# elicassion/active-gym

Hardware: NVIDIA B200
Metric: foveal_obs_per_sec (higher is better)
Workload: dtype u8

## Files before the change

### active_gym_b200/csrc/agym_device.cuh

```cuda
#pragma once
#include "agym_kernels.cuh"
#ifndef AGYM_EXPERIMENT
#define AGYM_EXPERIMENT 0
#endif

#include <cuda.h>
#include <cuda_bf16.h>
#include <cuda_fp16.h>

#include <algorithm>
#include <utility>
#include <cstdlib>
#include <cstring>

#include "../../include/agym_b200.h"

namespace agym {

namespace {


constexpr int kThreads = 256;

__device__ __forceinline__ uint4 ld_stream128(const void *p) {
// ... 176 lines not shown
                "selp.u32 %0, 1, 0, p;\n\t}"
                : "=r"(done)
                : "r"(smem_u32(bar)), "r"(parity)
                : "memory");
        }
    }
}
__device__ __forceinline__ void bulk_g2s(void *smem_dst, const void *gmem_src, uint32_t bytes, uint64_t *bar) {
    asm volatile("cp.async.bulk.shared::cluster.global.mbarrier::complete_tx::bytes [%0], [%1], %2, [%3];" ::"r"(
                     smem_u32(smem_dst)),
                 "l"(gmem_src), "r"(bytes), "r"(smem_u32(bar))
                 : "memory");
}

__device__ __forceinline__ void tensor_g2s_4d(void *smem_dst, const CUtensorMap *map, uint64_t *bar, int c0, int c1, int c2, int c3) {
    asm volatile("cp.async.bulk.tensor.4d.shared::cluster.global.mbarrier::complete_tx::bytes [%0], [%1, {%3, %4, %5, %6}], [%2];" ::"r"(
                     smem_u32(smem_dst)),
                 "l"(reinterpret_cast<uint64_t>(map)), "r"(smem_u32(bar)), "r"(c0), "r"(c1), "r"(c2), "r"(c3)
                 : "memory");
}

__device__ __forceinline__ void bulk_s2g(void *gmem_dst, const void *smem_src, uint32_t bytes) {
    asm volatile("cp.async.bulk.global.shared::cta.bulk_group [%0], [%1], %2;" ::"l"(gmem_dst), "r"(smem_u32(smem_src)),
                 "r"(bytes)
                 : "memory");
}
__device__ __forceinline__ void bulk_commit() { asm volatile("cp.async.bulk.commit_group;" ::: "memory"); }
template <int N>
__device__ __forceinline__ void bulk_wait_read() { asm volatile("cp.async.bulk.wait_group.read %0;" ::"n"(N) : "memory"); }
__device__ __forceinline__ void fence_async_smem() { asm volatile("fence.proxy.async.shared::cta;" ::: "memory"); }

__device__ __forceinline__ void mbar_arrive(uint64_t *bar) {
    asm volatile("mbarrier.arrive.shared::cta.b64 _, [%0];" ::"r"(smem_u32(bar)) : "memory");
}
__device__ __forceinline__ void consumer_sync() { asm volatile("bar.sync 1, %0;" ::"n"(kThreads) : "memory"); }

__device__ __forceinline__ void pdl_launch_dependents() { asm volatile("griddepcontrol.launch_dependents;" ::: "memory"); }
__device__ __forceinline__ void pdl_wait() { asm volatile("griddepcontrol.wait;" ::: "memory"); }

__device__ __forceinline__ void cp_async16(void *smem_dst, const void *gmem_src) {
    asm volatile("cp.async.cg.shared.global [%0], [%1], 16;" ::"r"((uint32_t)__cvta_generic_to_shared(smem_dst)), "l"(gmem_src));
}
__device__ __forceinline__ void cp_async16_s(uint32_t smem_addr, const void *gmem_src) {
    asm volatile("cp.async.cg.shared.global [%0], [%1], 16;" ::"r"(smem_addr), "l"(gmem_src));
}
__device__ __forceinline__ void cp_async4(void *smem_dst, const void *gmem_src) {
    asm volatile("cp.async.ca.shared.global [%0], [%1], 4;" ::"r"((uint32_t)__cvta_generic_to_shared(smem_dst)), "l"(gmem_src));
}
__device__ __forceinline__ void cp_async4_s(uint32_t smem_addr, const void *gmem_src) {
    asm volatile("cp.async.ca.shared.global [%0], [%1], 4;" ::"r"(smem_addr), "l"(gmem_src));
}
template <int SOFF, int GOFF>
__device__ __forceinline__ void cp_async4_imm(uint32_t smem_addr, const void *gmem_src) {
    asm volatile("cp.async.ca.shared.global [%0 + %2], [%1 + %3], 4;" ::"r"(smem_addr), "l"(gmem_src), "n"(SOFF), "n"(GOFF));
}
__device__ __forceinline__ void cp_async_commit() { asm volatile("cp.async.commit_group;" ::: "memory"); }
template <int N>
__device__ __forceinline__ void cp_async_wait() { asm volatile("cp.async.wait_group %0;" ::"n"(N) : "memory"); }

__device__ __forceinline__ float norm_u8(uint32_t u) {
    const float x = (float)u, r = 1.0f / 255.0f;
    const float q0 = x * r;
    return fmaf(fmaf(-q0, 255.0f, x), r, q0);
}
__device__ __forceinline__ void norm_store4(int dt, uint32_t word, void *dst, size_t index) {
    const float f0 = norm_u8(word & 0xffu), f1 = norm_u8((word >> 8) & 0xffu), f2 = norm_u8((word >> 16) & 0xffu), f3 = norm_u8(word >> 24);
    if (dt == AGYM_DTYPE_F32) {
        reinterpret_cast<float4 *>(dst)[index] = make_float4(f0, f1, f2, f3);
    } else if (dt == AGYM_DTYPE_F16) {
        const __half2 a = __floats2half2_rn(f0, f1), b = __floats2half2_rn(f2, f3);
        reinterpret_cast<uint2 *>(dst)[index] = make_uint2(*reinterpret_cast<const uint32_t *>(&a), *reinterpret_cast<const uint32_t *>(&b));
    } else {
        const __nv_bfloat162 a = __floats2bfloat162_rn(f0, f1), b = __floats2bfloat162_rn(f2, f3);
        reinterpret_cast<uint2 *>(dst)[index] = make_uint2(*reinterpret_cast<const uint32_t *>(&a), *reinterpret_cast<const uint32_t *>(&b));
    }
}
__device__ __forceinline__ void norm_store16(int dt, const uint4 v, void *dst, size_t index) {
    const uint32_t w[4] = {v.x, v.y, v.z, v.w};
    if (dt == AGYM_DTYPE_F32) {
        float4 *o = reinterpret_cast<float4 *>(dst) + 4 * index;
#pragma unroll
        for (int j = 0; j < 4; ++j)
            o[j] = make_float4(norm_u8(w[j] & 0xffu), norm_u8((w[j] >> 8) & 0xffu), norm_u8((w[j] >> 16) & 0xffu), norm_u8(w[j] >> 24));
    } else {
        uint32_t h[8];
#pragma unroll
        for (int j = 0; j < 4; ++j) {
            const float f0 = norm_u8(w[j] & 0xffu), f1 = norm_u8((w[j] >> 8) & 0xffu), f2 = norm_u8((w[j] >> 16) & 0xffu), f3 = norm_u8(w[j] >> 24);
            if (dt == AGYM_DTYPE_F16) {
                const __half2 a = __floats2half2_rn(f0, f1), b = __floats2half2_rn(f2, f3);
                h[2 * j] = *reinterpret_cast<const uint32_t *>(&a); h[2 * j + 1] = *reinterpret_cast<const uint32_t *>(&b);
            } else {
                const __nv_bfloat162 a = __floats2bfloat162_rn(f0, f1), b = __floats2bfloat162_rn(f2, f3);
                h[2 * j] = *reinterpret_cast<const uint32_t *>(&a); h[2 * j + 1] = *reinterpret_cast<const uint32_t *>(&b);
            }
        }
        uint4 *o = reinterpret_cast<uint4 *>(dst) + 2 * index;
        o[0] = make_uint4(h[0], h[1], h[2], h[3]);
        o[1] = make_uint4(h[4], h[5], h[6], h[7]);
    }
}

__device__ __forceinline__ uint64_t pack2(float lo, float hi) {
    uint64_t r;
    asm("mov.b64 %0, {%1, %2};" : "=l"(r) : "f"(lo), "f"(hi));
    return r;
}
__device__ __forceinline__ void unpack2(uint64_t v, uint32_t &lo, uint32_t &hi) {
    asm("mov.b64 {%0, %1}, %2;" : "=r"(lo), "=r"(hi) : "l"(v));
}
__device__ __forceinline__ uint64_t ffma2(uint64_t a, uint64_t b, uint64_t c) {
    uint64_t d;
    asm("fma.rn.f32x2 %0, %1, %2, %3;" : "=l"(d) : "l"(a), "l"(b), "l"(c));
    return d;
}
__device__ __forceinline__ uint64_t fsub2(uint64_t a, uint64_t b) {
    uint64_t d;
    asm("sub.rn.f32x2 %0, %1, %2;" : "=l"(d) : "l"(a), "l"(b));
    return d;
}
__device__ __forceinline__ uint64_t fadd2(uint64_t a, uint64_t b) {
    uint64_t d;
    asm("add.rn.f32x2 %0, %1, %2;" : "=l"(d) : "l"(a), "l"(b));
    return d;
}

template <typename F>
cudaError_t set_smem(F func, size_t bytes) {
    if (bytes > 48 * 1024)
        return cudaFuncSetAttribute(func, cudaFuncAttributeMaxDynamicSharedMemorySize, (int)bytes);
    return cudaSuccess;
}

size_t a16(size_t v) { return (v + 15) & ~size_t(15); }

const bool g_no_pdl = getenv("AGYM_NO_PDL") != nullptr;

template <typename... KArgs, typename... Args>
cudaError_t launch_pdl(void (*kern)(KArgs...), dim3 grid, dim3 block, size_t smem, cudaStream_t st, Args &&...args) {
    cudaLaunchConfig_t cfg = {};
    cfg.gridDim = grid; cfg.blockDim = block; cfg.dynamicSmemBytes = smem; cfg.stream = st;
    cudaLaunchAttribute at[1];
    at[0].id = cudaLaunchAttributeProgrammaticStreamSerialization;
    at[0].val.programmaticStreamSerializationAllowed = g_no_pdl ? 0 : 1;
    cfg.attrs = at; cfg.numAttrs = 1;
    return cudaLaunchKernelEx(&cfg, kern, KArgs(std::forward<Args>(args))...);
}

const bool g_disable_std = getenv("AGYM_NO_STD") != nullptr;
const bool g_disable_tma = getenv("AGYM_NO_TMA") != nullptr;
const bool g_flex_old = getenv("AGYM_FLEX_OLD") != nullptr;
const bool g_crop_old = getenv("AGYM_CROP_OLD") != nullptr;
const bool g_crop_v2 = getenv("AGYM_CROP_V2") != nullptr;
const bool g_std_nofs = getenv("AGYM_STD_NOFS") != nullptr;
const int g_units = getenv("AGYM_INGEST_UNITS") ? atoi(getenv("AGYM_INGEST_UNITS")) : 0;


}

}
```

### active_gym_b200/csrc/agym_observe.cu

```cuda
#include "agym_device.cuh"

namespace agym {

namespace {

template <int VARIANT>
__global__ void __launch_bounds__(kThreads) k_observe_fixed(const __grid_constant__ DevPlan p,
                                                            const uint8_t *__restrict__ ring,
                                                            const int32_t *__restrict__ head,
                                                            const double *__restrict__ action,
                                                            const uint8_t *__restrict__ ctrl, int32_t *__restrict__ loc,
                                                            uint8_t *__restrict__ out) {
    extern __shared__ __align__(16) uint8_t smem[];
    __shared__ int s_loc[2];
    const int n = blockIdx.x, tid = threadIdx.x;
    if (tid == 0) {
        int r, c;
        update_loc_fixed(p, n, action, ctrl, loc, r, c);
        s_loc[0] = r; s_loc[1] = c;
    }
    __syncthreads();
    const int r0 = s_loc[0], c0 = s_loc[1];
    const int h = head[n];
    const uint8_t *env_ring = ring + (size_t)n * p.K * p.plane;
// ... 395 lines not shown
    const int nw_max = (p.f_w + 3) / 4 + 1;
    const int sq_words = (K * pp + 3) & ~3, buf_words = sq_words + ((K * f_h * nw_max + 3) & ~3);
    const int trows = K * p.p_h;
    float *bufs = reinterpret_cast<float *>(smem);
    float *s_T = bufs + 2 * buf_words;
    int2 *s_row = reinterpret_cast<int2 *>(s_T + trows * S_w);
    const uint32_t *ring_w = reinterpret_cast<const uint32_t *>(ring);
    uint32_t *out_w = reinterpret_cast<uint32_t *>(out);
    const int G = gridDim.x;

    const int npairs = S_w >> 1, parts = nt / npairs;
    const int a_part = tid / npairs, cp = tid - a_part * npairs;
    const bool a_active = a_part < parts;
    int a_i0 = 0, a_i1 = 0;
    uint64_t a_w0 = 0, a_w1 = 0;
    if (a_active) {
        a_i0 = __ldg(p.exw_i0 + 2 * cp);
        a_i1 = __ldg(p.exw_i0 + 2 * cp + 1);
        a_w0 = pack2(__ldg(p.exw_w0 + 2 * cp), __ldg(p.exw_w0 + 2 * cp + 1));
        a_w1 = pack2(__ldg(p.exw_w1 + 2 * cp), __ldg(p.exw_w1 + 2 * cp + 1));
    }
    const uint64_t bias2 = pack2(kBias, kBias);
    const int g = tid / quads, q = tid - g * quads;
    const bool active = g < ysegs;
    const int rows_per = (p.S_h + ysegs - 1) / ysegs;
    const int y_begin = g * rows_per, y_end = active ? min(p.S_h, y_begin + rows_per) : y_begin;
    const int pp4 = pp >> 2, frows = K * f_h;
    for (int i = tid; i < p.S_h; i += nt) s_row[i] = make_int2(__ldg(p.exh_i0 + i), __float_as_int(__ldg(p.exh_w0 + i)));
    if (tid == 0) s_row[p.S_h] = make_int2(-1, 0);

    auto issue = [&](int env, int lr, int lc, int hh, int b) {
        float *sq = bufs + b * buf_words;
        uint32_t *fv = reinterpret_cast<uint32_t *>(sq + sq_words);
        const size_t slot0 = (size_t)env * K;
        for (int k = 0; k < K; ++k) {
            int slot = hh + 1 + k;
            slot -= slot >= K ? K : 0;
            const float *src = pcache + (slot0 + slot) * pp;
            for (int c = tid; c < pp4; c += nt) cp_async16(sq + k * pp + 4 * c, src + 4 * c);
        }
        const int wq0 = lc >> 2, nw = ((lc + p.f_w - 1) >> 2) - wq0 + 1;
        for (int r = tid; r < frows; r += nt) {
            const int k = r / f_h, yy = r - k * f_h;
            int slot = hh + 1 + k;
            slot -= slot >= K ? K : 0;
            const uint32_t *src = ring_w + (slot0 + slot) * wpp + (uint32_t)(lr + yy) * quads + wq0;
            uint32_t *dst = fv + r * nw_max;
            for (int w = 0; w < nw; ++w) cp_async4(dst + w, src + w);
        }
    };
    auto next_loc = [&](int env, int slot) {
        int r = 0, c = 0;
        if (env < N) update_loc_fixed<true>(p, env, action, ctrl, loc, r, c);
        s_loc[slot][0] = r;
        s_loc[slot][1] = c;
    };

    int e = blockIdx.x;
    if (tid == 0) { next_loc(e, 0); next_loc(e + G, 1); }
    __syncthreads();
    int lr = s_loc[0][0], lc = s_loc[0][1], lr1 = s_loc[1][0], lc1 = s_loc[1][1];
    int hh = 0, hh1 = 0;
    if (e < N) { hh = head[e]; issue(e, lr, lc, hh, 0); }
    cp_async_commit();
    if (e + G < N) hh1 = head[e + G];
    __syncthreads();

    for (int it = 0; e < N; e += G, ++it) {
        const int en = e + G;
        if (en < N) issue(en, lr1, lc1, hh1, (it + 1) & 1);
        cp_async_commit();
        if (tid == 0) next_loc(en + G, it & 1);
        int hh2 = 0;
        if (en + G < N) hh2 = head[en + G];
        cp_async_wait<1>();
        __syncthreads();

        const float *sq = bufs + (it & 1) * buf_words;
        if (a_active) {
            const float *s = sq + a_part * p.p_w;
            float *t = s_T + a_part * S_w + 2 * cp;
            const int sstep = parts * p.p_w, tstep = parts * S_w;
#pragma unroll 4
            for (int r = a_part; r < trows; r += parts, s += sstep, t += tstep) {
                const uint64_t u = pack2(s[a_i0], s[a_i1]), v = pack2(s[a_i0 + 1], s[a_i1 + 1]);
                *reinterpret_cast<uint64_t *>(t) = ffma2(a_w0, u, ffma2(a_w1, v, bias2));
            }
        }
        __syncthreads();

        if (active) {
            const uint32_t *fvb = reinterpret_cast<const uint32_t *>(sq + sq_words);
            const uint32_t fov_mask = word_mask(4 * q, lc, lc + p.f_w);
            const int rf = fov_mask ? lr : (1 << 29);
            const int fstride = f_h * nw_max;
            for (int k0 = 0; k0 < K; k0 += KG) {
                uint32_t *orow = out_w + ((size_t)e * K + k0) * wpp + (uint32_t)y_begin * quads + q;
                const uint32_t *fv = fvb + (k0 * f_h - rf) * nw_max + (q - (lc >> 2));
                const float *tk = s_T + (size_t)k0 * p.p_h * S_w + 4 * q;
                const int kstride = p.p_h * S_w;
                int y = y_begin, j_have = -2;
                const int2 *rp = s_row + y_begin;
                int2 rw = *rp;
                uint64_t b0[KG], b1[KG], d0[KG], d1[KG];
                while (y < y_end) {
                    const int j0 = rw.x;
#pragma unroll
                    for (int kk = 0; kk < KG; ++kk) {
                        const float *tj = tk + kk * kstride + j0 * S_w;
                        uint64_t a0, a1;
                        if (j0 == j_have + 1) { a0 = b0[kk]; a1 = b1[kk]; }
                        else { const ulonglong2 a = *reinterpret_cast<const ulonglong2 *>(tj); a0 = a.x; a1 = a.y; }
                        const ulonglong2 b = *reinterpret_cast<const ulonglong2 *>(tj + S_w);
                        b0[kk] = b.x; b1[kk] = b.y;
                        d0[kk] = fsub2(a0, b.x); d1[kk] = fsub2(a1, b.y);
                    }
                    j_have = j0;
                    do {
                        const float w0 = __int_as_float(rw.y);
                        const uint64_t w2 = pack2(w0, w0);
                        rw = *++rp;
                        uint32_t word[KG];
#pragma unroll
                        for (int kk = 0; kk < KG; ++kk) {
                            uint32_t u0, u1, u2, u3;
                            unpack2(ffma2(w2, d0[kk], b0[kk]), u0, u1);
                            unpack2(ffma2(w2, d1[kk], b1[kk]), u2, u3);
                            word[kk] = __byte_perm(__byte_perm(u0, u1, 0x0051), __byte_perm(u2, u3, 0x0051), 0x5410);
                        }
                        if ((unsigned)(y - rf) < (unsigned)f_h) {
                            const uint32_t *sh = fv + y * nw_max;
#pragma unroll
                            for (int kk = 0; kk < KG; ++kk) word[kk] = (word[kk] & ~fov_mask) | (sh[kk * fstride] & fov_mask);
                        }
#pragma unroll
                        for (int kk = 0; kk < KG; ++kk) orow[kk * wpp] = word[kk];
                        orow += quads;
                        ++y;
                    } while (rw.x == j0 && y < y_end);
                }
            }
        }
        __syncthreads();
        lr = lr1; lc = lc1; hh = hh1; hh1 = hh2;
        lr1 = s_loc[it & 1][0]; lc1 = s_loc[it & 1][1];
    }
}

struct StdGeom {
    static constexpr int S = 84, P = 20, Q = 21, SEG = 4, R = 21, SPAN = 7;
    __host__ __device__ static constexpr int src(int i) { return (40 * i - 64 + 168 * 4) / 168 - 4; }
};

template <int NW, int R0>
__device__ __forceinline__ void prefetch_rows_imm(uint32_t rows, uint32_t dst, const uint32_t *src) {
    if constexpr (R0 < StdGeom::R) {
        if (rows & (1u << R0)) cp_async4_imm<R0 * (NW ? NW : 1) * 4, R0 * StdGeom::Q * 4>(dst, src);
        prefetch_rows_imm<NW, R0 + 1>(rows, dst, src);
    }
}

template <int K, int NW, bool FS>
__global__ void __launch_bounds__(((StdGeom::Q * StdGeom::SEG * K + 31) / 32) * 32, 2)
    k_observe_peripheral_std(const __grid_constant__ DevPlan p, const __grid_constant__ ExpandStd ew,
                             const uint8_t *__restrict__ ring, const int32_t *__restrict__ head,
                             const float *__restrict__ pcache, const double *__restrict__ action,
                             const uint8_t *__restrict__ ctrl, int32_t *__restrict__ loc, uint8_t *__restrict__ out) {
    using Gm = StdGeom;
    constexpr int S = Gm::S, P = Gm::P, Q = Gm::Q, R = Gm::R;
    constexpr int NB = Q * Gm::SEG * K;
    constexpr int PP = P * P, PLANE_W = S * S / 4;
    constexpr int NBUF = 3, DIST = 2, LOC_RING = 128;
    extern __shared__ __align__(16) uint8_t smem[];
    __shared__ int4 s_loc[LOC_RING];
    __shared__ __align__(8) uint64_t full[NBUF];
    const int tid = threadIdx.x;
    const int N = p.N, f_h = p.f_h, f_w = p.f_w, G = gridDim.x;
    const int nw_max = NW ? NW : (f_w + 3) / 4 + 1;
    const int rowbuf = (f_h * Q + 9) & ~3;
    const int buf_words = K * PP + (FS ? K * rowbuf : ((K * f_h * nw_max + 3) & ~3));
    float *bufs = reinterpret_cast<float *>(smem);
    uint32_t *tiles = reinterpret_cast<uint32_t *>(bufs + NBUF * buf_words);
    const uint32_t *ring_w = reinterpret_cast<const uint32_t *>(ring);

    auto loc_batch = [&](int it0) {
        const int j = it0 + (tid & 31);
        const int env = j <= N / G + 1 ? (int)blockIdx.x + j * G : N;
        int r = 0, c = 0, hh = 0;
        if (env < N) {
            update_loc_fixed<true>(p, env, action, ctrl, loc, r, c);
            hh = head[env];
        }
        s_loc[j & (LOC_RING - 1)] = make_int4(r, c, hh, 0);
    };
    pdl_launch_dependents();
    if (tid == 0) {
        for (int i = 0; i < NBUF; ++i) mbar_init(&full[i], 1);
        mbar_fence_init();
    }

    const bool active = tid < NB;
    const int q = tid % Q, t2 = tid / Q;
    constexpr int kOrd4[16] = {7, 4, 13, 3, 0, 1, 9, 6, 10, 14, 11, 12, 8, 5, 15, 2};
    constexpr int kOrd3[12] = {11, 8, 5, 2, 9, 6, 3, 0, 10, 4, 1, 7};
    const int grp = !active ? 0 : (K == 4 ? kOrd4[t2 & 15] : (K == 3 ? kOrd3[t2 % 12] : t2));
    const int g = grp % Gm::SEG, k = grp / Gm::SEG;
    int base;
    uint64_t wa01, wa23, wb01, wb23, wc01, wc23;
    {
        const int i00 = __ldg(p.exw_i0 + 4 * q);
        base = min(i00, P - 3);
        float wa[4], wb[4], wc[4];
#pragma unroll
        for (int c = 0; c < 4; ++c) {
            const int sel = __ldg(p.exw_i0 + 4 * q + c) - base;
            const float w0 = __ldg(p.exw_w0 + 4 * q + c), w1 = __ldg(p.exw_w1 + 4 * q + c);
            wa[c] = sel == 0 ? w0 : 0.f;
            wb[c] = sel == 0 ? w1 : w0;
            wc[c] = sel == 0 ? 0.f : w1;
        }
        wa01 = pack2(wa[0], wa[1]); wa23 = pack2(wa[2], wa[3]);
        wb01 = pack2(wb[0], wb[1]); wb23 = pack2(wb[2], wb[3]);
        wc01 = pack2(wc[0], wc[1]); wc23 = pack2(wc[2], wc[3]);
    }
    const uint64_t bias2 = pack2(kBias, kBias);
    const int row_first = 5 * g - 1;
    const int so_t0 = (row_first < 0 ? 0 : row_first) * P + base;
    const int so_mid = row_first * P + base;
    const int so_t6 = (row_first + 6 > P - 1 ? P - 1 : row_first + 6) * P + base;
    const uint32_t bufs_s = smem_u32(bufs);
    const uint32_t word0 = (uint32_t)(g * R) * Q + q;
    constexpr int NJ = 2;
    int ck_row[NJ], ck_k[NJ], ck_c4[NJ];
    if constexpr (FS) {
        const int cpr = (f_w + 14) / 16 + 1, total = K * f_h * cpr;
#pragma unroll
        for (int a = 0; a < NJ; ++a) {
            const int i = tid + a * (int)blockDim.x;
            const int row = i / cpr, kk = row / f_h;
            ck_k[a] = i < total ? kk : -1;
            ck_row[a] = (row - kk * f_h) * Q;
            ck_c4[a] = (i - row * cpr) * 4;
        }
    }

    auto fovea_rows = [&](int lr, int lc, uint32_t &mask) {
        mask = word_mask(4 * q, lc, lc + f_w);
        const int r_lo = lr - g * R;
        const int m_lo = max(r_lo, 0), m_hi = min(r_lo + f_h, R);
        return (mask && m_hi > m_lo) ? (((1u << m_hi) - 1u) & ~((1u << m_lo) - 1u)) : 0u;
    };
    auto fovea_pos = [&](int lr, int lc) { return (k * f_h + g * R - lr) * nw_max + (q - (lc >> 2)); };
    auto prefetch = [&](int env, int j) {
        const int b = j % NBUF;
        if (tid == 0) {
            mbar_expect_tx(&full[b], K * PP * 4);
            bulk_g2s(bufs + b * buf_words, pcache + (size_t)env * (K * PP), K * PP * 4, &full[b]);
        }
        if constexpr (FS) {
            const int4 lh = s_loc[j & (LOC_RING - 1)];
            const int top = lh.x * Q, wb = top & ~3;
            const int lw = lh.y >> 2, lastw = (lh.y + f_w - 1) >> 2;
#pragma unroll
            for (int a = 0; a < NJ; ++a) {
                if (ck_k[a] < 0) continue;
                const int rowbase = top + ck_row[a];
                const int cw = ((rowbase + lw) & ~3) + ck_c4[a];
                if (cw > rowbase + lastw) continue;
                int slot = lh.z + 1 + ck_k[a];
                slot -= slot >= K ? K : 0;
                cp_async16_s(bufs_s + (uint32_t)(b * buf_words + K * PP + ck_k[a] * rowbuf + (cw - wb)) * 4u,
                             ring_w + ((size_t)env * K + slot) * PLANE_W + cw);
            }
        } else if (active) {
            const int4 lh = s_loc[j & (LOC_RING - 1)];
            uint32_t mask;
            const uint32_t rows = fovea_rows(lh.x, lh.y, mask);
            if (rows) {
                int slot = lh.z + 1 + k;
                slot -= slot >= K ? K : 0;
                const uint32_t *src = ring_w + ((size_t)env * K + slot) * PLANE_W + word0;
                const uint32_t dst = bufs_s + (uint32_t)(b * buf_words + K * PP + fovea_pos(lh.x, lh.y)) * 4u;
                if (NW) {
                    prefetch_rows_imm<NW, 0>(rows, dst, src);
                } else {
#pragma unroll
                    for (int r = 0; r < R; ++r)
                        if (rows & (1u << r)) cp_async4_s(dst + (uint32_t)(r * nw_max) * 4u, src + r * Q);
                }
            }
        }
    };
    auto t_row = [&](const float *sq, int so, uint64_t &t01, uint64_t &t23) {
        const float s0 = sq[so], s1 = sq[so + 1], s2 = sq[so + 2];
        const uint64_t p0 = pack2(s0, s0), p1 = pack2(s1, s1), p2 = pack2(s2, s2);
        t01 = ffma2(p2, wc01, ffma2(p1, wb01, ffma2(p0, wa01, bias2)));
        t23 = ffma2(p2, wc23, ffma2(p1, wb23, ffma2(p0, wa23, bias2)));
    };

    pdl_wait();
    if (tid < 32) loc_batch(0);
    __syncthreads();
    {
        const int e0 = blockIdx.x;
#pragma unroll
        for (int j = 0; j < DIST; ++j) {
            if (e0 + j * G < N) prefetch(e0 + j * G, j);
            cp_async_commit();
        }
        if constexpr (FS) {
            cp_async_wait<DIST - 1>();
            __syncthreads();
        }
    }
    int it = 0;
    for (int e = blockIdx.x; e < N; e += G, ++it) {
        if (e + DIST * G < N) prefetch(e + DIST * G, it + DIST);
        cp_async_commit();
        if ((it & 31) == 0 && tid < 32) loc_batch(it + 32);
        const int b = it % NBUF;
        if constexpr (!FS) cp_async_wait<DIST>();
        mbar_wait(&full[b], (it / NBUF) & 1);
        uint32_t *tile = tiles + (it & 1) * (K * PLANE_W);
        if (active) {
            const int4 lh = s_loc[it & (LOC_RING - 1)];
            uint32_t fov_mask;
            const uint32_t rows = fovea_rows(lh.x, lh.y, fov_mask);
            int slot = lh.z + 1 + k;
            slot -= slot >= K ? K : 0;
            const float *sq = bufs + b * buf_words + slot * PP;
            const uint32_t *sh = reinterpret_cast<const uint32_t *>(bufs + b * buf_words + K * PP) +
                                 (FS ? k * rowbuf + (int)word0 - ((lh.x * Q) & ~3) : fovea_pos(lh.x, lh.y));
            constexpr int SHP = FS ? Q : 0;
            uint32_t *o = tile + k * PLANE_W + word0;
            uint64_t a0, a1, b0, b1, d0 = 0, d1 = 0;
            t_row(sq, so_t0, a0, a1);
            t_row(sq, so_mid + P, b0, b1);
            int t_have = 0;
#pragma unroll
            for (int r = 0; r < R; ++r) {
                const int t = Gm::src(r) + 1;
                if (t != t_have) {
                    a0 = b0; a1 = b1;
                    t_row(sq, t + 1 == Gm::SPAN - 1 ? so_t6 : so_mid + (t + 1) * P, b0, b1);
                    t_have = t;
                }
                if (r == 0 || Gm::src(r) != Gm::src(r - 1)) { d0 = fsub2(a0, b0); d1 = fsub2(a1, b1); }
                const uint64_t w2 = pack2(ew.hw[r], ew.hw[r]);
                uint32_t u0, u1, u2, u3;
                unpack2(ffma2(w2, d0, b0), u0, u1);
                unpack2(ffma2(w2, d1, b1), u2, u3);
                uint32_t word = __byte_perm(__byte_perm(u0, u1, 0x0051), __byte_perm(u2, u3, 0x0051), 0x5410);
                if (rows & (1u << r))
                    word = (word & ~fov_mask) | (sh[FS ? r * SHP : r * nw_max] & fov_mask);
                o[r * Q] = word;
            }
        }
        fence_async_smem();
        if (tid == 0) bulk_wait_read<0>();
        if constexpr (FS) cp_async_wait<DIST - 1>();
        __syncthreads();
        if (tid == 0) {
            bulk_s2g(out + (size_t)e * (K * PLANE_W * 4), tile, K * PLANE_W * 4);
            bulk_commit();
        }
        if (p.norm_out) {
            const uint4 *t4 = reinterpret_cast<const uint4 *>(tile);
            for (int i = tid; i < K * PLANE_W / 4; i += (int)blockDim.x)
                norm_store16(p.norm_dt, t4[i], p.norm_out, (size_t)e * (K * PLANE_W / 4) + i);
        }
    }
    if (tid == 0) bulk_wait_read<0>();
}


}

namespace {
cudaError_t normalize_after(cudaError_t e, const uint8_t *out, size_t bytes, void *norm_out, int norm_dt, cudaStream_t st) {
    if (e != cudaSuccess || !norm_out) return e;
    if (bytes % 16 != 0) return cudaErrorInvalidValue;
    return launch_normalize(out, bytes, norm_dt, norm_out, st);
}
}

cudaError_t launch_observe_fixed(const DevPlan &p0, const uint8_t *ring, const int32_t *head, const double *action,
                                 const uint8_t *ctrl, int32_t *loc, int variant, uint8_t *out, void *norm_out, int norm_dt,
                                 cudaStream_t st) {
    DevPlan p = p0;
    p.norm_out = norm_out; p.norm_dt = norm_dt;
    const size_t out_bytes = (size_t)p.N * p.K * (variant == AGYM_OUT_CROP ? p.f_h * p.f_w : p.plane);
    cudaError_t e;
    const int crop_nwx = (p.f_w + 2) / 4 + 1;
    const size_t crop_smem = a16((size_t)(p.K * p.f_h * p.f_w / 4) * 8) + (size_t)kCropWarps * p.K * p.f_h * crop_nwx * 4;
    CropV3Args c3;
    c3.nch = (p.f_w + 30) / 16;
    c3.g = p.f_w % 4 == 0 ? 1 : p.f_w % 2 == 0 ? 2 : 4;
    c3.gw = c3.g * p.f_w / 4;
    c3.ngroups = p.K * p.f_h / c3.g;
    c3.m_fh = 0xFFFFFFFFu / (uint32_t)p.f_h + 1u;
    c3.slice = (int)(16 + (size_t)p.K * p.f_h * c3.nch * 16);
    const int c3_warps = (p.C == 3 && (size_t)kCrop3Warps * (c3.slice + (size_t)p.K * p.f_h * p.f_w) > 100 * 1024) ? 4 : kCrop3Warps;
    const size_t crop3_smem = (size_t)c3_warps * (c3.slice + (size_t)p.K * p.f_h * p.f_w);
    if (variant == AGYM_OUT_CROP && (p.K * p.f_h * p.f_w) % 4 == 0 && (p.K * p.f_h) % c3.g == 0 && p.plane % 16 == 0 &&
        (reinterpret_cast<uintptr_t>(ring) & 15) == 0 && (reinterpret_cast<uintptr_t>(out) & 3) == 0 &&
        !g_disable_std && !g_crop_old && !g_crop_v2 && crop3_smem <= 100 * 1024) {
        const int grid = (p.N + c3_warps - 1) / c3_warps;
#define AGYM_LAUNCH_CROP3(FW, W)                                                                                  \
    {                                                                                                             \
        if ((e = set_smem(k_observe_fixed_crop_v3<FW, W>, crop3_smem)) != cudaSuccess) return e;                   \
        k_observe_fixed_crop_v3<FW, W><<<grid, W * 32, crop3_smem, st>>>(p, ring, head, action, ctrl, loc, out, c3); \
    }
        if (c3_warps == 4) {
            if (p.f_w == 30) AGYM_LAUNCH_CROP3(30, 4)
            else AGYM_LAUNCH_CROP3(0, 4)
        } else if (p.f_w == 30) AGYM_LAUNCH_CROP3(30, kCrop3Warps)
        else AGYM_LAUNCH_CROP3(0, kCrop3Warps)
#undef AGYM_LAUNCH_CROP3
        return cudaGetLastError();
    }
    if (variant == AGYM_OUT_CROP && (p.K * p.f_h * p.f_w) % 4 == 0 && !g_disable_std && !g_crop_old &&
        crop_smem <= 64 * 1024 && p.K * p.f_h * crop_nwx * 4 + 4 < 65536) {
        if ((e = set_smem(k_observe_fixed_crop_v2, crop_smem)) != cudaSuccess) return e;
        k_observe_fixed_crop_v2<<<(p.N + kCropWarps - 1) / kCropWarps, kCropWarps * 32, crop_smem, st>>>(p, ring, head, action, ctrl, loc, out, crop_nwx);
        return cudaGetLastError();
    } else if (variant == AGYM_OUT_CROP && (p.K * p.f_h * p.f_w) % 4 == 0 && !g_disable_std) {
        k_observe_fixed_crop_warp<<<(p.N + kThreads / 32 - 1) / (kThreads / 32), kThreads, 0, st>>>(p, ring, head, action, ctrl, loc, out);
    } else if (variant == AGYM_OUT_CROP) {
        k_observe_fixed<AGYM_OUT_CROP><<<p.N, kThreads, 0, st>>>(p, ring, head, action, ctrl, loc, out);
    } else if (variant == AGYM_OUT_MASK) {
        k_observe_fixed<AGYM_OUT_MASK><<<p.N, kThreads, 0, st>>>(p, ring, head, action, ctrl, loc, out);
    } else {
        const size_t smem = sizeof(float) * ((size_t)p.f_h * p.f_w + (size_t)p.f_h * p.S_w);
        if ((e = set_smem(k_observe_fixed<AGYM_OUT_RESIZE_FULL>, smem)) != cudaSuccess) return e;
        k_observe_fixed<AGYM_OUT_RESIZE_FULL><<<p.N, kThreads, smem, st>>>(p, ring, head, action, ctrl, loc, out);
    }
    return normalize_after(cudaGetLastError(), out, out_bytes, norm_out, norm_dt, st);
}

cudaError_t launch_observe_peripheral(const DevPlan &p0, const ExpandStd *ew, const uint8_t *ring, const int32_t *head,
                                      const float *pcache, const double *action, const uint8_t *ctrl, int32_t *loc,
                                      uint8_t *out, void *norm_out, int norm_dt, cudaStream_t st) {
    DevPlan p = p0;
    p.norm_out = norm_out; p.norm_dt = norm_dt;
    const size_t out_bytes = (size_t)p.N * p.K * p.plane;
    const size_t smem = a16(p.plane) + sizeof(float) * ((size_t)p.S_h * p.p_w + (size_t)p.p_h * p.p_w + (size_t)p.p_h * p.S_w);
    cudaError_t e;
    const int quads = p.S_w / 4;
    if (pcache && ew && ew->ok && (p.K == 4 || p.K == 3) && !g_disable_std && p.N < (1 << 30) &&
        (reinterpret_cast<uintptr_t>(out) & 15) == 0 && (reinterpret_cast<uintptr_t>(pcache) & 15) == 0) {
        const int nw_max = (p.f_w + 3) / 4 + 1;
        const size_t fov_words = ((size_t)p.K * p.f_h * nw_max + 3) & ~size_t(3);
        size_t fs = 4 * (3 * ((size_t)p.K * 400 + fov_words) + 2 * (size_t)p.K * 1764);
        const size_t fs_rows = 4 * (3 * ((size_t)p.K * 400 + (size_t)p.K * ((p.f_h * 21 + 9) & ~3)) + 2 * (size_t)p.K * 1764);
        const int std_threads = ((21 * 4 * p.K + 31) / 32) * 32;
        const bool full_rows = !g_std_nofs && fs_rows <= 112 * 1024 && p.K * p.f_h * ((p.f_w + 14) / 16 + 1) <= 2 * std_threads;
        int dev = 0, sms = 148, occ = 0;
        cudaGetDevice(&dev);
        cudaDeviceGetAttribute(&sms, cudaDevAttrMultiProcessorCount, dev);
#define AGYM_LAUNCH_STD(KK, NW, FSV)                                                                               \
    {                                                                                                              \
    if (fs <= 220 * 1024) {                                                                                        \
        const int threads = ((21 * 4 * KK + 31) / 32) * 32;                                                        \
        if ((e = set_smem(k_observe_peripheral_std<KK, NW, FSV>, fs)) != cudaSuccess) return e;                    \
        cudaOccupancyMaxActiveBlocksPerMultiprocessor(&occ, k_observe_peripheral_std<KK, NW, FSV>, threads, fs);   \
        if (occ >= 1) {                                                                                            \
            return launch_pdl(k_observe_peripheral_std<KK, NW, FSV>, dim3(std::min(p.N, sms * occ)), dim3(threads), fs, st, \
                              p, *ew, ring, head, pcache, action, ctrl, loc, out);                                 \
        }                                                                                                          \
    }                                                                                                              \
    }
        if (full_rows) {
            fs = fs_rows;
            if (p.K == 4) AGYM_LAUNCH_STD(4, 0, true)
            else AGYM_LAUNCH_STD(3, 0, true)
        }
        else if (p.K == 4 && nw_max == 9) AGYM_LAUNCH_STD(4, 9, false)
        else if (p.K == 4) AGYM_LAUNCH_STD(4, 0, false)
        else if (nw_max == 9) AGYM_LAUNCH_STD(3, 9, false)
        else AGYM_LAUNCH_STD(3, 0, false)
#undef AGYM_LAUNCH_STD
    }
    if (pcache && p.fast_expand && quads <= 64 && (p.p_h * p.p_w) % 4 == 0) {
        int ysegs = std::max(1, 128 / quads);
        {
            int g = p.S_h, b2 = p.p_h;
            while (b2) { const int t = g % b2; g = b2; b2 = t; }
            const int period = p.S_h / g;
            while (ysegs > 1 && (p.S_h % ysegs != 0 || (p.S_h / ysegs) % period != 0)) --ysegs;
        }
        const int threads = ((std::max(quads * ysegs, 2 * quads) + 31) / 32) * 32;
        const int nw_max = (p.f_w + 3) / 4 + 1;
        const size_t buf_words = (((size_t)p.K * p.p_h * p.p_w + 3) & ~size_t(3)) + (((size_t)p.K * p.f_h * nw_max + 3) & ~size_t(3));
        const size_t fs = 4 * (2 * buf_words + (size_t)p.K * p.p_h * p.S_w) + 8 * ((size_t)p.S_h + 1);
        int dev = 0, sms = 148, occ = 1;
        cudaGetDevice(&dev);
        cudaDeviceGetAttribute(&sms, cudaDevAttrMultiProcessorCount, dev);
#define AGYM_LAUNCH_PF(KG, PW)                                                                                     \
    {                                                                                                              \
        if ((e = set_smem(k_observe_peripheral_v2<KG, PW>, fs)) != cudaSuccess) return e;                          \
        cudaOccupancyMaxActiveBlocksPerMultiprocessor(&occ, k_observe_peripheral_v2<KG, PW>, threads, fs);         \
        if (occ < 1) return cudaErrorInvalidConfiguration;                                                         \
        k_observe_peripheral_v2<KG, PW><<<std::min(p.N, sms * occ), threads, fs, st>>>(p, ring, head, pcache, action, \
                                                                                      ctrl, loc, out, ysegs);     \
    }
        if (p.K == 4 && p.plane == 7056) AGYM_LAUNCH_PF(4, 1764)
        else if (p.K == 3 && p.plane == 7056) AGYM_LAUNCH_PF(3, 1764)
        else if (p.C == 3 && p.K % 3 == 0 && p.plane == 7056) AGYM_LAUNCH_PF(3, 1764)
        else if (p.K % 4 == 0) AGYM_LAUNCH_PF(4, 0)
        else if (p.K % 3 == 0) AGYM_LAUNCH_PF(3, 0)
        else if (p.K % 2 == 0) AGYM_LAUNCH_PF(2, 0)
        else AGYM_LAUNCH_PF(1, 0)
#undef AGYM_LAUNCH_PF
        return normalize_after(cudaGetLastError(), out, out_bytes, norm_out, norm_dt, st);
    }
    if (pcache) {
        if ((e = set_smem(k_observe_peripheral<true>, smem)) != cudaSuccess) return e;
        k_observe_peripheral<true><<<p.N, kThreads, smem, st>>>(p, ring, head, pcache, action, ctrl, loc, out);
    } else {
        if ((e = set_smem(k_observe_peripheral<false>, smem)) != cudaSuccess) return e;
        k_observe_peripheral<false><<<p.N, kThreads, smem, st>>>(p, ring, head, pcache, action, ctrl, loc, out);
    }
    return normalize_after(cudaGetLastError(), out, out_bytes, norm_out, norm_dt, st);
}


}
```

Before: 51.58 million.

## Replace per-env peripheral std kernel with per-plane 96-thread pipelined kernel

The templated per-environment kernel, which processed all K frame planes in one block of 21*4*K threads, is replaced by a single non-templated kernel. Each 96-thread block handles one plane at a time and runs a TMA and cp.async prefetch pipeline over (env, plane) pairs. This shrinks shared memory per block and allows up to 8 blocks per SM, and it extends the fast path to K=9 with C=3. Lanes are assigned to output words so that a warp's stores fall on distinct banks. The trade-offs are more pipeline stages and barriers per env, one bulk store per plane, and the PDL launch-dependents trigger moving to the end of the kernel, which may reduce overlap with the next kernel.

```diff
diff --git a/active_gym_b200/csrc/agym_device.cuh b/active_gym_b200/csrc/agym_device.cuh
--- a/active_gym_b200/csrc/agym_device.cuh
+++ b/active_gym_b200/csrc/agym_device.cuh
@@ -352,7 +352,6 @@
 const bool g_flex_old = getenv("AGYM_FLEX_OLD") != nullptr;
 const bool g_crop_old = getenv("AGYM_CROP_OLD") != nullptr;
 const bool g_crop_v2 = getenv("AGYM_CROP_V2") != nullptr;
-const bool g_std_nofs = getenv("AGYM_STD_NOFS") != nullptr;
 const int g_units = getenv("AGYM_INGEST_UNITS") ? atoi(getenv("AGYM_INGEST_UNITS")) : 0;
 
 
diff --git a/active_gym_b200/csrc/agym_observe.cu b/active_gym_b200/csrc/agym_observe.cu
--- a/active_gym_b200/csrc/agym_observe.cu
+++ b/active_gym_b200/csrc/agym_observe.cu
@@ -571,33 +571,23 @@
     __host__ __device__ static constexpr int src(int i) { return (40 * i - 64 + 168 * 4) / 168 - 4; }
 };
 
-template <int NW, int R0>
-__device__ __forceinline__ void prefetch_rows_imm(uint32_t rows, uint32_t dst, const uint32_t *src) {
-    if constexpr (R0 < StdGeom::R) {
-        if (rows & (1u << R0)) cp_async4_imm<R0 * (NW ? NW : 1) * 4, R0 * StdGeom::Q * 4>(dst, src);
-        prefetch_rows_imm<NW, R0 + 1>(rows, dst, src);
-    }
-}
-
-template <int K, int NW, bool FS>
-__global__ void __launch_bounds__(((StdGeom::Q * StdGeom::SEG * K + 31) / 32) * 32, 2)
-    k_observe_peripheral_std(const __grid_constant__ DevPlan p, const __grid_constant__ ExpandStd ew,
-                             const uint8_t *__restrict__ ring, const int32_t *__restrict__ head,
-                             const float *__restrict__ pcache, const double *__restrict__ action,
-                             const uint8_t *__restrict__ ctrl, int32_t *__restrict__ loc, uint8_t *__restrict__ out) {
+constexpr int kPlaneThreads = 96;
+__global__ void __launch_bounds__(kPlaneThreads, 8)
+    k_observe_peripheral_planes(const __grid_constant__ DevPlan p, const __grid_constant__ ExpandStd ew,
+                                const uint8_t *__restrict__ ring, const int32_t *__restrict__ head,
+                                const float *__restrict__ pcache, const double *__restrict__ action,
+                                const uint8_t *__restrict__ ctrl, int32_t *__restrict__ loc, uint8_t *__restrict__ out) {
     using Gm = StdGeom;
     constexpr int S = Gm::S, P = Gm::P, Q = Gm::Q, R = Gm::R;
-    constexpr int NB = Q * Gm::SEG * K;
     constexpr int PP = P * P, PLANE_W = S * S / 4;
-    constexpr int NBUF = 3, DIST = 2, LOC_RING = 128;
+    constexpr int NBUF = 3, DIST = 2, LOC_RING = 64;
     extern __shared__ __align__(16) uint8_t smem[];
     __shared__ int4 s_loc[LOC_RING];
     __shared__ __align__(8) uint64_t full[NBUF];
     const int tid = threadIdx.x;
-    const int N = p.N, f_h = p.f_h, f_w = p.f_w, G = gridDim.x;
-    const int nw_max = NW ? NW : (f_w + 3) / 4 + 1;
+    const int N = p.N, K = p.K, f_h = p.f_h, f_w = p.f_w, G = gridDim.x;
     const int rowbuf = (f_h * Q + 9) & ~3;
-    const int buf_words = K * PP + (FS ? K * rowbuf : ((K * f_h * nw_max + 3) & ~3));
+    const int buf_words = PP + rowbuf;
     float *bufs = reinterpret_cast<float *>(smem);
     uint32_t *tiles = reinterpret_cast<uint32_t *>(bufs + NBUF * buf_words);
     const uint32_t *ring_w = reinterpret_cast<const uint32_t *>(ring);
@@ -612,18 +602,21 @@
         }
         s_loc[j & (LOC_RING - 1)] = make_int4(r, c, hh, 0);
     };
-    pdl_launch_dependents();
     if (tid == 0) {
         for (int i = 0; i < NBUF; ++i) mbar_init(&full[i], 1);
         mbar_fence_init();
     }
 
-    const bool active = tid < NB;
-    const int q = tid % Q, t2 = tid / Q;
-    constexpr int kOrd4[16] = {7, 4, 13, 3, 0, 1, 9, 6, 10, 14, 11, 12, 8, 5, 15, 2};
-    constexpr int kOrd3[12] = {11, 8, 5, 2, 9, 6, 3, 0, 10, 4, 1, 7};
-    const int grp = !active ? 0 : (K == 4 ? kOrd4[t2 & 15] : (K == 3 ? kOrd3[t2 % 12] : t2));
-    const int g = grp % Gm::SEG, k = grp / Gm::SEG;
+    const int warp = tid >> 5, lane = tid & 31;
+    int item = -1;
+    {
+        int seen = 0;
+#pragma unroll
+        for (int i = 0; i < Q * Gm::SEG; ++i)
+            if ((i / Q * R * Q + i % Q) % 32 == lane && seen++ == warp) item = i;
+    }
+    const bool active = item >= 0;
+    const int q = active ? item % Q : 0, g = active ? item / Q : 0;
     int base;
     uint64_t wa01, wa23, wb01, wb23, wc01, wc23;
     {
@@ -649,19 +642,8 @@
     const int so_t6 = (row_first + 6 > P - 1 ? P - 1 : row_first + 6) * P + base;
     const uint32_t bufs_s = smem_u32(bufs);
     const uint32_t word0 = (uint32_t)(g * R) * Q + q;
-    constexpr int NJ = 2;
-    int ck_row[NJ], ck_k[NJ], ck_c4[NJ];
-    if constexpr (FS) {
-        const int cpr = (f_w + 14) / 16 + 1, total = K * f_h * cpr;
-#pragma unroll
-        for (int a = 0; a < NJ; ++a) {
-            const int i = tid + a * (int)blockDim.x;
-            const int row = i / cpr, kk = row / f_h;
-            ck_k[a] = i < total ? kk : -1;
-            ck_row[a] = (row - kk * f_h) * Q;
-            ck_c4[a] = (i - row * cpr) * 4;
-        }
-    }
+    const int cpr = (f_w + 14) / 16 + 1, chunks = f_h * cpr;
+    const FastDiv fd_cpr(cpr);
 
     auto fovea_rows = [&](int lr, int lc, uint32_t &mask) {
         mask = word_mask(4 * q, lc, lc + f_w);
@@ -669,45 +651,24 @@
         const int m_lo = max(r_lo, 0), m_hi = min(r_lo + f_h, R);
         return (mask && m_hi > m_lo) ? (((1u << m_hi) - 1u) & ~((1u << m_lo) - 1u)) : 0u;
     };
-    auto fovea_pos = [&](int lr, int lc) { return (k * f_h + g * R - lr) * nw_max + (q - (lc >> 2)); };
-    auto prefetch = [&](int env, int j) {
-        const int b = j % NBUF;
+    auto prefetch = [&](int ie, int k, int jb) {
+        const int b = jb % NBUF;
+        const int4 lh = s_loc[ie & (LOC_RING - 1)];
+        int slot = lh.z + 1 + k;
+        slot -= slot >= K ? K : 0;
+        const size_t plane = (size_t)((int)blockIdx.x + ie * G) * K + slot;
         if (tid == 0) {
-            mbar_expect_tx(&full[b], K * PP * 4);
-            bulk_g2s(bufs + b * buf_words, pcache + (size_t)env * (K * PP), K * PP * 4, &full[b]);
-        }
-        if constexpr (FS) {
-            const int4 lh = s_loc[j & (LOC_RING - 1)];
-            const int top = lh.x * Q, wb = top & ~3;
-            const int lw = lh.y >> 2, lastw = (lh.y + f_w - 1) >> 2;
-#pragma unroll
-            for (int a = 0; a < NJ; ++a) {
-                if (ck_k[a] < 0) continue;
-                const int rowbase = top + ck_row[a];
-                const int cw = ((rowbase + lw) & ~3) + ck_c4[a];
-                if (cw > rowbase + lastw) continue;
-                int slot = lh.z + 1 + ck_k[a];
-                slot -= slot >= K ? K : 0;
-                cp_async16_s(bufs_s + (uint32_t)(b * buf_words + K * PP + ck_k[a] * rowbuf + (cw - wb)) * 4u,
-                             ring_w + ((size_t)env * K + slot) * PLANE_W + cw);
-            }
-        } else if (active) {
-            const int4 lh = s_loc[j & (LOC_RING - 1)];
-            uint32_t mask;
-            const uint32_t rows = fovea_rows(lh.x, lh.y, mask);
-            if (rows) {
-                int slot = lh.z + 1 + k;
-                slot -= slot >= K ? K : 0;
-                const uint32_t *src = ring_w + ((size_t)env * K + slot) * PLANE_W + word0;
-                const uint32_t dst = bufs_s + (uint32_t)(b * buf_words + K * PP + fovea_pos(lh.x, lh.y)) * 4u;
-                if (NW) {
-                    prefetch_rows_imm<NW, 0>(rows, dst, src);
-                } else {
-#pragma unroll
-                    for (int r = 0; r < R; ++r)
-                        if (rows & (1u << r)) cp_async4_s(dst + (uint32_t)(r * nw_max) * 4u, src + r * Q);
-                }
-            }
+            mbar_expect_tx(&full[b], PP * 4);
+            bulk_g2s(bufs + b * buf_words, pcache + plane * PP, PP * 4, &full[b]);
+        }
+        const int top = lh.x * Q, wb = top & ~3;
+        const int lw = lh.y >> 2, lastw = (lh.y + f_w - 1) >> 2;
+        for (int i = tid; i < chunks; i += kPlaneThreads) {
+            const int row = fd_cpr.div(i);
+            const int rowbase = top + row * Q;
+            const int cw = ((rowbase + lw) & ~3) + (i - row * cpr) * 4;
+            if (cw <= rowbase + lastw)
+                cp_async16_s(bufs_s + (uint32_t)(b * buf_words + PP + (cw - wb)) * 4u, ring_w + plane * PLANE_W + cw);
         }
     };
     auto t_row = [&](const float *sq, int so, uint64_t &t01, uint64_t &t23) {
@@ -720,75 +681,71 @@
     pdl_wait();
     if (tid < 32) loc_batch(0);
     __syncthreads();
-    {
-        const int e0 = blockIdx.x;
-#pragma unroll
-        for (int j = 0; j < DIST; ++j) {
-            if (e0 + j * G < N) prefetch(e0 + j * G, j);
-            cp_async_commit();
-        }
-        if constexpr (FS) {
+    int pe = 0, pk = 0;
+    auto prefetch_next = [&](int jb) {
+        if ((int)blockIdx.x + pe * G < N) prefetch(pe, pk, jb);
+        cp_async_commit();
+        if (++pk == K) { pk = 0; ++pe; }
+    };
+#pragma unroll
+    for (int j = 0; j < DIST; ++j) prefetch_next(j);
+    cp_async_wait<DIST - 1>();
+    __syncthreads();
+    int jb = 0;
+    for (int ie = 0, e = blockIdx.x; e < N; e += G, ++ie) {
+        const int4 lh = s_loc[ie & (LOC_RING - 1)];
+        uint32_t fov_mask;
+        const uint32_t rows = fovea_rows(lh.x, lh.y, fov_mask);
+        for (int k = 0; k < K; ++k, ++jb) {
+            prefetch_next(jb + DIST);
+            if (k == 0 && (ie & 31) == 0 && tid < 32) loc_batch(ie + 32);
+            const int b = jb % NBUF;
+            mbar_wait(&full[b], (jb / NBUF) & 1);
+            uint32_t *tile = tiles + (jb & 1) * PLANE_W;
+            if (active) {
+                const float *sq = bufs + b * buf_words;
+                const uint32_t *sh = reinterpret_cast<const uint32_t *>(sq + PP) + (int)word0 - ((lh.x * Q) & ~3);
+                uint32_t *o = tile + word0;
+                uint64_t a0, a1, b0, b1, d0 = 0, d1 = 0;
+                t_row(sq, so_t0, a0, a1);
+                t_row(sq, so_mid + P, b0, b1);
+                int t_have = 0;
+#pragma unroll
+                for (int r = 0; r < R; ++r) {
+                    const int t = Gm::src(r) + 1;
+                    if (t != t_have) {
+                        a0 = b0; a1 = b1;
+                        t_row(sq, t + 1 == Gm::SPAN - 1 ? so_t6 : so_mid + (t + 1) * P, b0, b1);
+                        t_have = t;
+                    }
+                    if (r == 0 || Gm::src(r) != Gm::src(r - 1)) { d0 = fsub2(a0, b0); d1 = fsub2(a1, b1); }
+                    const uint64_t w2 = pack2(ew.hw[r], ew.hw[r]);
+                    uint32_t u0, u1, u2, u3;
+                    unpack2(ffma2(w2, d0, b0), u0, u1);
+                    unpack2(ffma2(w2, d1, b1), u2, u3);
+                    uint32_t word = __byte_perm(__byte_perm(u0, u1, 0x0051), __byte_perm(u2, u3, 0x0051), 0x5410);
+                    if (rows & (1u << r))
+                        word = (word & ~fov_mask) | (sh[r * Q] & fov_mask);
+                    o[r * Q] = word;
+                }
+            }
+            fence_async_smem();
+            if (tid == 0) bulk_wait_read<0>();
             cp_async_wait<DIST - 1>();
             __syncthreads();
-        }
-    }
-    int it = 0;
-    for (int e = blockIdx.x; e < N; e += G, ++it) {
-        if (e + DIST * G < N) prefetch(e + DIST * G, it + DIST);
-        cp_async_commit();
-        if ((it & 31) == 0 && tid < 32) loc_batch(it + 32);
-        const int b = it % NBUF;
-        if constexpr (!FS) cp_async_wait<DIST>();
-        mbar_wait(&full[b], (it / NBUF) & 1);
-        uint32_t *tile = tiles + (it & 1) * (K * PLANE_W);
-        if (active) {
-            const int4 lh = s_loc[it & (LOC_RING - 1)];
-            uint32_t fov_mask;
-            const uint32_t rows = fovea_rows(lh.x, lh.y, fov_mask);
-            int slot = lh.z + 1 + k;
-            slot -= slot >= K ? K : 0;
-            const float *sq = bufs + b * buf_words + slot * PP;
-            const uint32_t *sh = reinterpret_cast<const uint32_t *>(bufs + b * buf_words + K * PP) +
-                                 (FS ? k * rowbuf + (int)word0 - ((lh.x * Q) & ~3) : fovea_pos(lh.x, lh.y));
-            constexpr int SHP = FS ? Q : 0;
-            uint32_t *o = tile + k * PLANE_W + word0;
-            uint64_t a0, a1, b0, b1, d0 = 0, d1 = 0;
-            t_row(sq, so_t0, a0, a1);
-            t_row(sq, so_mid + P, b0, b1);
-            int t_have = 0;
-#pragma unroll
-            for (int r = 0; r < R; ++r) {
-                const int t = Gm::src(r) + 1;
-                if (t != t_have) {
-                    a0 = b0; a1 = b1;
-                    t_row(sq, t + 1 == Gm::SPAN - 1 ? so_t6 : so_mid + (t + 1) * P, b0, b1);
-                    t_have = t;
-                }
-                if (r == 0 || Gm::src(r) != Gm::src(r - 1)) { d0 = fsub2(a0, b0); d1 = fsub2(a1, b1); }
-                const uint64_t w2 = pack2(ew.hw[r], ew.hw[r]);
-                uint32_t u0, u1, u2, u3;
-                unpack2(ffma2(w2, d0, b0), u0, u1);
-                unpack2(ffma2(w2, d1, b1), u2, u3);
-                uint32_t word = __byte_perm(__byte_perm(u0, u1, 0x0051), __byte_perm(u2, u3, 0x0051), 0x5410);
-                if (rows & (1u << r))
-                    word = (word & ~fov_mask) | (sh[FS ? r * SHP : r * nw_max] & fov_mask);
-                o[r * Q] = word;
-            }
-        }
-        fence_async_smem();
-        if (tid == 0) bulk_wait_read<0>();
-        if constexpr (FS) cp_async_wait<DIST - 1>();
-        __syncthreads();
-        if (tid == 0) {
-            bulk_s2g(out + (size_t)e * (K * PLANE_W * 4), tile, K * PLANE_W * 4);
-            bulk_commit();
-        }
-        if (p.norm_out) {
-            const uint4 *t4 = reinterpret_cast<const uint4 *>(tile);
-            for (int i = tid; i < K * PLANE_W / 4; i += (int)blockDim.x)
-                norm_store16(p.norm_dt, t4[i], p.norm_out, (size_t)e * (K * PLANE_W / 4) + i);
-        }
-    }
+            const size_t plane_out = (size_t)e * K + k;
+            if (tid == 0) {
+                bulk_s2g(out + plane_out * (PLANE_W * 4), tile, PLANE_W * 4);
+                bulk_commit();
+            }
+            if (p.norm_out) {
+                const uint4 *t4 = reinterpret_cast<const uint4 *>(tile);
+                for (int i = tid; i < PLANE_W / 4; i += kPlaneThreads)
+                    norm_store16(p.norm_dt, t4[i], p.norm_out, plane_out * (PLANE_W / 4) + i);
+            }
+        }
+    }
+    pdl_launch_dependents();
     if (tid == 0) bulk_wait_read<0>();
 }
 
@@ -866,39 +823,17 @@
     const size_t smem = a16(p.plane) + sizeof(float) * ((size_t)p.S_h * p.p_w + (size_t)p.p_h * p.p_w + (size_t)p.p_h * p.S_w);
     cudaError_t e;
     const int quads = p.S_w / 4;
-    if (pcache && ew && ew->ok && (p.K == 4 || p.K == 3) && !g_disable_std && p.N < (1 << 30) &&
+    if (pcache && ew && ew->ok && (p.K == 4 || p.K == 3 || (p.C == 3 && p.K == 9)) && !g_disable_std && p.N < (1 << 30) &&
         (reinterpret_cast<uintptr_t>(out) & 15) == 0 && (reinterpret_cast<uintptr_t>(pcache) & 15) == 0) {
-        const int nw_max = (p.f_w + 3) / 4 + 1;
-        const size_t fov_words = ((size_t)p.K * p.f_h * nw_max + 3) & ~size_t(3);
-        size_t fs = 4 * (3 * ((size_t)p.K * 400 + fov_words) + 2 * (size_t)p.K * 1764);
-        const size_t fs_rows = 4 * (3 * ((size_t)p.K * 400 + (size_t)p.K * ((p.f_h * 21 + 9) & ~3)) + 2 * (size_t)p.K * 1764);
-        const int std_threads = ((21 * 4 * p.K + 31) / 32) * 32;
-        const bool full_rows = !g_std_nofs && fs_rows <= 112 * 1024 && p.K * p.f_h * ((p.f_w + 14) / 16 + 1) <= 2 * std_threads;
+        const size_t fs = 4 * (3 * (400 + (size_t)((p.f_h * 21 + 9) & ~3)) + 2 * 1764);
         int dev = 0, sms = 148, occ = 0;
         cudaGetDevice(&dev);
         cudaDeviceGetAttribute(&sms, cudaDevAttrMultiProcessorCount, dev);
-#define AGYM_LAUNCH_STD(KK, NW, FSV)                                                                               \
-    {                                                                                                              \
-    if (fs <= 220 * 1024) {                                                                                        \
-        const int threads = ((21 * 4 * KK + 31) / 32) * 32;                                                        \
-        if ((e = set_smem(k_observe_peripheral_std<KK, NW, FSV>, fs)) != cudaSuccess) return e;                    \
-        cudaOccupancyMaxActiveBlocksPerMultiprocessor(&occ, k_observe_peripheral_std<KK, NW, FSV>, threads, fs);   \
-        if (occ >= 1) {                                                                                            \
-            return launch_pdl(k_observe_peripheral_std<KK, NW, FSV>, dim3(std::min(p.N, sms * occ)), dim3(threads), fs, st, \
-                              p, *ew, ring, head, pcache, action, ctrl, loc, out);                                 \
-        }                                                                                                          \
-    }                                                                                                              \
-    }
-        if (full_rows) {
-            fs = fs_rows;
-            if (p.K == 4) AGYM_LAUNCH_STD(4, 0, true)
-            else AGYM_LAUNCH_STD(3, 0, true)
-        }
-        else if (p.K == 4 && nw_max == 9) AGYM_LAUNCH_STD(4, 9, false)
-        else if (p.K == 4) AGYM_LAUNCH_STD(4, 0, false)
-        else if (nw_max == 9) AGYM_LAUNCH_STD(3, 9, false)
-        else AGYM_LAUNCH_STD(3, 0, false)
-#undef AGYM_LAUNCH_STD
+        if ((e = set_smem(k_observe_peripheral_planes, fs)) != cudaSuccess) return e;
+        cudaOccupancyMaxActiveBlocksPerMultiprocessor(&occ, k_observe_peripheral_planes, kPlaneThreads, fs);
+        if (occ >= 1)
+            return launch_pdl(k_observe_peripheral_planes, dim3(std::min(p.N, sms * occ)), dim3(kPlaneThreads), fs, st,
+                              p, *ew, ring, head, pcache, action, ctrl, loc, out);
     }
     if (pcache && p.fast_expand && quads <= 64 && (p.p_h * p.p_w) % 4 == 0) {
         int ysegs = std::max(1, 128 / quads);
```

Result: faster. 52.71 million, median of 6 (+2.2%).
